# finsberg/fenicsx-beat

Hardware: AMD Instinct MI355X
Metric: node_updates_per_sec (higher is better)
Workload: dtype f64

## Files before the change

### fenicsx-beat_amd/csrc/beat_ode.hip

```cpp
#include "beat_ode_kernel.h"
#include "beat_ode_jit.h"

#include <functional>


template <class Model>
static int launch_ode_run(beat_ctx* ctx, double* states, int64_t n, int64_t ld, const double* host_params,
                          int num_params, const double* ppn, int64_t pld, double t0, double dt, int64_t nsteps,
                          int nbeats, int save_freq, const int* track_idx, int ntrack, double* trace) {
  BEAT_REQUIRE(num_params == Model::NP || (host_params == nullptr && ppn == nullptr && Model::NP == 2),
               "model expects %d parameters, got %d", Model::NP, num_params);
  BEAT_REQUIRE(ntrack >= 0 && ntrack <= 8, "at most 8 tracked states");
  BEAT_REQUIRE(ntrack == 0 || (trace != nullptr && save_freq >= 1), "tracking needs a trace buffer and save_freq >= 1");
  ParamPack<Model::NP> prm;
  for (int k = 0; k < Model::NP; ++k) prm.p[k] = host_params ? host_params[k] : 1.0;
  typename Model::Derived drv = Model::derive(prm.p);
  TrackSpec tr{};
  tr.n = ntrack;
  for (int a = 0; a < ntrack; ++a) {
    BEAT_REQUIRE(track_idx[a] >= 0 && track_idx[a] < Model::NS, "tracked state %d out of range", track_idx[a]);
    tr.idx[a] = track_idx[a];
  }
  const unsigned grid = (unsigned)((n + BEAT_BLOCK - 1) / BEAT_BLOCK);
  if (ppn != nullptr) {
    BEAT_REQUIRE(pld >= n, "params_ld %lld < n %lld", (long long)pld, (long long)n);
    BEAT_KERNEL((ode_run_kernel<Model, true>), dim3(grid), dim3(BEAT_BLOCK), 0, ctx->stream, states, n, ld, prm,
                       drv, ppn, pld, t0, dt, nsteps, nbeats, save_freq, tr, trace);
  } else {
    BEAT_KERNEL((ode_run_kernel<Model, false>), dim3(grid), dim3(BEAT_BLOCK), 0, ctx->stream, states, n, ld,
                       prm, drv, ppn, pld, t0, dt, nsteps, nbeats, save_freq, tr, trace);
  }
  BEAT_LAUNCH_CHECK();
  return BEAT_OK;
}

template <class M> struct ModelTag { using type = M; };
constexpr int BEAT_NOT_BUILTIN = 1001;

template <class F>
static int with_builtin_model(int model_id, F&& f) {
  switch (model_id) {
    case BEAT_MODEL_SIMPLE_ODE: return f(ModelTag<SimpleOde>{});
    case BEAT_MODEL_FHN_DEMO: return f(ModelTag<FhnDemo>{});
    case BEAT_MODEL_FHN_README: return f(ModelTag<FhnReadme>{});
    case BEAT_MODEL_TP06_GRL1: return f(ModelTag<Tp06Grl1>{});
    case BEAT_MODEL_TORORD_DYNCL_GRL1: return f(ModelTag<TorordDynClGrl1>{});
    case BEAT_MODEL_TORORD_LAND_GRL1: return f(ModelTag<TorordLandGrl1>{});
    default: return BEAT_NOT_BUILTIN;
  }
}

static int unknown_model(int model_id) {
  beat_set_error("unknown model id %d", model_id);
  return BEAT_EINVAL;
}

extern "C" int beat_ode_run(beat_ctx* ctx, int model_id, double* dev_states, int64_t n, int64_t ld,
                            const double* host_params, int num_params, const double* dev_params_per_node,
                            int64_t params_ld, double t0, double dt, int64_t nsteps, int nbeats, int save_freq,
                            const int* host_track_idx, int ntrack, double* dev_trace) {
  BEAT_REQUIRE(ctx != nullptr && dev_states != nullptr, "null argument");
  BEAT_REQUIRE(n >= 0 && ld >= n && nsteps >= 0 && nbeats >= 0, "bad shape");
  if (n == 0 || nsteps == 0 || nbeats == 0) return BEAT_OK;
  if (model_id >= BEAT_MODEL_CUSTOM_BASE)
    return beat_custom_run(ctx, model_id, dev_states, n, ld, host_params, num_params, dev_params_per_node, params_ld, t0, dt, nsteps, nbeats,
                           save_freq, host_track_idx, ntrack, dev_trace);
  const int rc = with_builtin_model(model_id, [&](auto tag) {
    return launch_ode_run<typename decltype(tag)::type>(ctx, dev_states, n, ld, host_params, num_params, dev_params_per_node, params_ld, t0, dt,
                                                        nsteps, nbeats, save_freq, host_track_idx, ntrack, dev_trace);
  });
  return rc == BEAT_NOT_BUILTIN ? unknown_model(model_id) : rc;
}

static unsigned ode_grid(int64_t n, int num_states) {
  unsigned grid = (unsigned)((n + BEAT_BLOCK - 1) / BEAT_BLOCK);
  static const int grid_cap_env = [] {
    const char* e = std::getenv("BEAT_ODE_GRID");
    return e ? std::atoi(e) : -1;
  }();
  static const int tile_min_states = [] {
    const char* e = std::getenv("BEAT_ODE_TILE_MIN_STATES");
    return e ? std::atoi(e) : 12;
  }();
  const int grid_cap = grid_cap_env >= 0 ? grid_cap_env : (num_states >= tile_min_states ? 0 : 24576);
  static const bool balance = [] {
    const char* e = std::getenv("BEAT_ODE_BALANCE");
    return !(e && e[0] == '0');
  }();
  if (grid_cap > 0 && grid > (unsigned)grid_cap) {
    const unsigned per_block = (grid + (unsigned)grid_cap - 1) / (unsigned)grid_cap;
    grid = (balance && per_block <= 8) ? (grid + per_block - 1) / per_block : (unsigned)grid_cap;
  }
  return grid;
}

template <class Model, bool PER_NODE, bool MARKED = false, bool SPARSE = false>
static auto launch_instance(bool have_pend, hipStream_t stream, unsigned grid, double* states, int64_t n, int64_t ld,
                            const ParamPack<Model::NP>& prm, const typename Model::Derived& drv, const double* ppn, int64_t pld, double t,
                            double dt, int v_index, double* v_copy, const PendingV& pend, const MarkedArgs& mk, const SparseRows& sp) {
  if (have_pend)
    BEAT_KERNEL((ode_step_kernel<Model, PER_NODE, true, MARKED, SPARSE>), dim3(grid), dim3(BEAT_BLOCK), 0, stream, states, n, ld, prm, drv,
                ppn, pld, t, dt, v_index, v_copy, pend, mk, sp);
  else
    BEAT_KERNEL((ode_step_kernel<Model, PER_NODE, false, MARKED, SPARSE>), dim3(grid), dim3(BEAT_BLOCK), 0, stream, states, n, ld, prm, drv,
                ppn, pld, t, dt, v_index, v_copy, pend, mk, sp);
}

template <class Model>
static int launch_ode(beat_ctx* ctx, double* states, int64_t n, int64_t ld, const double* host_params,
                      int num_params, const double* ppn, int64_t pld, double t, double dt,
                      int v_index, double* v_copy, const PendingV& pend, MarkedArgs mk = MarkedArgs{nullptr, nullptr, 0, nullptr, nullptr},
                      SparseRows sp = SparseRows{{0}, 0}) {
  BEAT_REQUIRE(num_params == Model::NP || (host_params == nullptr && ppn == nullptr && Model::NP == 2) || mk.markers != nullptr,
               "model expects %d parameters, got %d", Model::NP, num_params);
  BEAT_REQUIRE(host_params != nullptr || ppn != nullptr || mk.markers != nullptr || Model::NP == 2,
               "no parameters given: a host vector, per-node rows or parameter classes");
  if (int rc = beat_check_step_rows(Model::NS, Model::V_INDEX, v_index, v_copy, mk.markers != nullptr, pend)) return rc;
  const bool have_pend = beat_pending_has_work(pend);
  ParamPack<Model::NP> prm;
  for (int k = 0; k < Model::NP; ++k) prm.p[k] = host_params ? host_params[k] : 1.0;
  typename Model::Derived drv = Model::derive(prm.p);
  const unsigned grid = ode_grid(n, Model::NS);
  if (mk.markers != nullptr) {
    BEAT_REQUIRE(ppn == nullptr && mk.table != nullptr, "parameter classes come with a table, not with per-node rows");
    launch_instance<Model, false, true>(have_pend, ctx->stream, grid, states, n, ld, prm, drv, ppn, pld, t, dt, v_index, v_copy, pend, mk, sp);
  } else if (ppn != nullptr && sp.count > 0) {
    BEAT_REQUIRE(pld >= n, "params_ld %lld < n %lld", (long long)pld, (long long)n);
    BEAT_REQUIRE(host_params != nullptr, "sparse rows come with the uniform parameter vector");
    {
      const int rc = beat_ode_jit_launch<Model>(ctx, dim3(grid), have_pend, states, n, ld, prm, drv, ppn, pld, t, dt, v_index, v_copy, pend, mk, sp);
      if (rc != BEAT_JIT_UNAVAILABLE) return rc;
    }
    BEAT_REQUIRE(sp.count <= BEAT_MAX_SPARSE_ROWS_RT, "%d varying rows need run-time compilation, which is not available here "
                 "(beat_ode_jit_stats; at most %d rows otherwise): pass all rows (beat_ode_step)", sp.count, BEAT_MAX_SPARSE_ROWS_RT);
    launch_instance<Model, true, false, true>(have_pend, ctx->stream, grid, states, n, ld, prm, drv, ppn, pld, t, dt, v_index, v_copy, pend, mk,
                                              sp);
  } else if (ppn != nullptr) {
    BEAT_REQUIRE(pld >= n, "params_ld %lld < n %lld", (long long)pld, (long long)n);
    launch_instance<Model, true>(have_pend, ctx->stream, grid, states, n, ld, prm, drv, ppn, pld, t, dt, v_index, v_copy, pend, mk, sp);
  } else {
    launch_instance<Model, false>(have_pend, ctx->stream, grid, states, n, ld, prm, drv, ppn, pld, t, dt, v_index, v_copy, pend, mk, sp);
  }
  BEAT_LAUNCH_CHECK();
  return BEAT_OK;
}

extern "C" int beat_ode_model_info(int model_id, int* num_states, int* num_params) {
  int ns = 0, np = 0;
  const int rc = with_builtin_model(model_id, [&](auto tag) {
    using M = typename decltype(tag)::type;
    ns = M::NS;
    np = M::NP;
    return BEAT_OK;
  });
  if (rc == BEAT_NOT_BUILTIN && beat_custom_model_info(model_id, &ns, &np, nullptr) != BEAT_OK)
    return unknown_model(model_id);
  if (num_states) *num_states = ns;
  if (num_params) *num_params = np;
  return BEAT_OK;
}

static int ode_step_dispatch(beat_ctx* ctx, int model_id, double* dev_states, int64_t n, int64_t ld,
                             const double* host_params, int num_params, const double* dev_params_per_node,
                             int64_t params_ld, double t, double dt, int v_index, double* dev_v_copy,
                             const PendingV& pend, MarkedArgs mk = MarkedArgs{nullptr, nullptr, 0, nullptr, nullptr},
                             SparseRows sp = SparseRows{{0}, 0}) {
  BEAT_REQUIRE(ctx != nullptr, "null context");
  BEAT_REQUIRE(dev_states != nullptr, "null states");
  BEAT_REQUIRE(n >= 0 && ld >= n, "bad shape n=%lld ld=%lld", (long long)n, (long long)ld);
  BEAT_REQUIRE((n + BEAT_BLOCK - 1) / BEAT_BLOCK < (int64_t)0x7fffffff, "n too large");
  if (n == 0) return BEAT_OK;
  if (model_id >= BEAT_MODEL_CUSTOM_BASE) {
    BEAT_REQUIRE(sp.count == 0, "a model registered as source takes a uniform vector, all per-node rows or classes (no sparse rows)");
    int cns = 0, cnp = 0, cvi = 0;
    if (int rc = beat_custom_model_info(model_id, &cns, &cnp, &cvi)) return rc;
    return beat_custom_step(ctx, model_id, ode_grid(n, cns), dev_states, n, ld, host_params, num_params, dev_params_per_node, params_ld, t, dt,
                            v_index, dev_v_copy, pend, mk);
  }
  const int rc = with_builtin_model(model_id, [&](auto tag) {
    return launch_ode<typename decltype(tag)::type>(ctx, dev_states, n, ld, host_params, num_params, dev_params_per_node, params_ld, t, dt,
                                                    v_index, dev_v_copy, pend, mk, sp);
  });
  return rc == BEAT_NOT_BUILTIN ? unknown_model(model_id) : rc;
}

extern "C" int beat_ode_step(beat_ctx* ctx, int model_id, double* dev_states, int64_t n, int64_t ld,
                             const double* host_params, int num_params,
                             const double* dev_params_per_node, int64_t params_ld, double t, double dt,
                             int v_index, double* dev_v_copy) {
  return ode_step_dispatch(ctx, model_id, dev_states, n, ld, host_params, num_params, dev_params_per_node, params_ld,
                           t, dt, v_index, dev_v_copy, PendingV{nullptr, 0, nullptr, 0, {}});
}

static int flush_long_ring(beat_pde* pde, double* v_row, const double* dev_ring0, int64_t field_stride, int& pending) {
  if (pending <= BEAT_MAX_PENDING) return BEAT_OK;
  pending = 0;
  return beat_pde_x_flush_terms(pde, nullptr, v_row, dev_ring0, field_stride, pde->last_base, 0, pde->guess.take_pending());
}

static int step_behind_open_solve(beat_ctx* ctx, beat_pde* pde, const double* dev_ring0, int64_t field_stride, int64_t n, double* v_row,
                                  const std::function<int(const PendingV&)>& launch) {
  BEAT_REQUIRE(pde != nullptr && pde->open.on, "pending = -1 needs an operator with an open solve");
  BEAT_REQUIRE(dev_ring0 != nullptr && field_stride >= n, "bad pending update");
  BEAT_REQUIRE(pde->open.x == v_row, "the open solve does not work on this row");
  PendingV behind{dev_ring0, field_stride, pde->d_alphas, 0, pde->guess.cur, pde->d_st, pde->ring};
  if (int rc = launch(behind)) return rc;
  beat_ksp_info info{};
  int pend2[2] = {0, 0};
  bool needed_more = false;
  const int rc_solve = beat_solve_end(pde, 1, &info, pend2, &needed_more);
  if (rc_solve != BEAT_OK && rc_solve != BEAT_ENOTCONV) return rc_solve;
  pde->guess.applied_behind = false;
  if (!needed_more) {
    pde->guess.pending_applied_behind();
    return BEAT_OK;
  }
  return launch(PendingV{dev_ring0, field_stride, pend2[1] ? pde->d_alphas : nullptr, pend2[1], pde->guess.take_pending(), nullptr, 0});
}

static int step_with_pending(beat_ctx* ctx, beat_pde* pde, double* v_row, int64_t n, const double* dev_ring0, int64_t field_stride,
                             int pending, bool long_ring, bool node_map, const std::function<int(const PendingV&)>& launch) {
  static_assert(BEAT_MAX_PENDING == beat_pde_detail::PRING && BEAT_MAX_PENDING_CLASS == beat_pde_detail::PRING_MAX, "pending directions = ring size");
  if (pending == -1) {
    BEAT_REQUIRE(long_ring || (pde != nullptr && pde->ring <= BEAT_MAX_PENDING),
                 "this kernel's pending path takes %d directions: finish the solve first", BEAT_MAX_PENDING);
    return step_behind_open_solve(ctx, pde, dev_ring0, field_stride, node_map ? 0 : n, v_row, launch);
  }
  BEAT_REQUIRE(pending >= 0 && pending <= BEAT_MAX_PENDING_CLASS, "pending count %d out of range", pending);
  BEAT_REQUIRE(pending == 0 || (pde != nullptr && dev_ring0 != nullptr && (field_stride >= n || node_map)), "bad pending update");
  BEAT_REQUIRE(pde == nullptr || !pde->open.on, "the operator has an open solve: finish it (beat_pde_solve_end) or pass pending = -1");
  if (!long_ring)
    if (int rc = flush_long_ring(pde, v_row, dev_ring0, field_stride, pending)) return rc;
  PendingV pend{dev_ring0, field_stride, pending ? pde->d_alphas : nullptr, pending, {}};
  if (pde != nullptr) pend.gt = pde->guess.take_pending();
  return launch(pend);
}

extern "C" int beat_ode_step_pending(beat_ctx* ctx, int model_id, double* dev_states, int64_t n, int64_t ld,
                                     const double* host_params, int num_params,
                                     const double* dev_params_per_node, int64_t params_ld, double t, double dt,
                                     int v_index, double* dev_v_copy, beat_pde* pde, const double* dev_ring0,
                                     int64_t field_stride, int pending) {
  double* v_row = dev_states + (int64_t)v_index * ld;
  return step_with_pending(ctx, pde, v_row, n, dev_ring0, field_stride, pending, false, false,
                           [&](const PendingV& pv) {
    return ode_step_dispatch(ctx, model_id, dev_states, n, ld, host_params, num_params, dev_params_per_node, params_ld, t, dt, v_index,
                             dev_v_copy, pv);
  });
}


extern "C" int beat_ode_step_rows(beat_ctx* ctx, int model_id, double* dev_states, int64_t n, int64_t ld,
                                  const double* host_params, int num_params, const int* host_row_params, int num_rows,
                                  const double* dev_rows, int64_t rows_ld, double t, double dt, int v_index, double* dev_v_copy,
                                  beat_pde* pde, const double* dev_ring0, int64_t field_stride, int pending) {
  BEAT_REQUIRE(host_params != nullptr && host_row_params != nullptr && dev_rows != nullptr, "null argument");
  BEAT_REQUIRE(num_rows >= 1 && num_rows <= BEAT_MAX_SPARSE_ROWS, "1..%d varying rows, got %d", BEAT_MAX_SPARSE_ROWS, num_rows);
  BEAT_REQUIRE(num_rows <= BEAT_MAX_SPARSE_ROWS_RT || beat_jit_enabled(), "%d varying rows need run-time compilation, which is not available "
               "here (beat_ode_jit_stats; at most %d rows otherwise): pass all rows (beat_ode_step)", num_rows, BEAT_MAX_SPARSE_ROWS_RT);
  SparseRows sp{{0}, num_rows};
  for (int j = 0; j < num_rows; ++j) {
    BEAT_REQUIRE(host_row_params[j] >= 0 && host_row_params[j] < num_params, "row %d names parameter %d of %d", j, host_row_params[j], num_params);
    sp.idx[j] = host_row_params[j];
  }
  double* v_row = dev_states + (int64_t)v_index * ld;
  return step_with_pending(ctx, pde, v_row, n, dev_ring0, field_stride, pending, false, false,
                           [&](const PendingV& pv) {
    return ode_step_dispatch(ctx, model_id, dev_states, n, ld, host_params, num_params, dev_rows, rows_ld, t, dt, v_index, dev_v_copy, pv,
                             MarkedArgs{nullptr, nullptr, 0, nullptr, nullptr}, sp);
  });
}

template <class Model>
static int fill_table(const double* host_params, int num_params, int classes, std::vector<double>& out) {
  BEAT_REQUIRE(num_params == Model::NP, "model expects %d parameters, got %d", Model::NP, num_params);
  static_assert(sizeof(OdeTableEntry<Model>) % sizeof(double) == 0, "table entry is a whole number of doubles");
  const size_t stride = sizeof(OdeTableEntry<Model>) / sizeof(double);
  out.assign(stride * (size_t)classes, 0.0);
  for (int c = 0; c < classes; ++c) {
    OdeTableEntry<Model>* e = (OdeTableEntry<Model>*)(out.data() + stride * c);
    for (int k = 0; k < Model::NP; ++k) e->p[k] = host_params[(size_t)c * Model::NP + k];
    e->d = Model::derive(e->p);
  }
  return BEAT_OK;
}

extern "C" int beat_ode_class_table_doubles(int model_id, int* doubles_per_class) {
  BEAT_REQUIRE(doubles_per_class != nullptr, "null argument");
  const int rc = with_builtin_model(model_id, [&](auto tag) {
    *doubles_per_class = (int)(sizeof(OdeTableEntry<typename decltype(tag)::type>) / sizeof(double));
    return BEAT_OK;
  });
  if (rc != BEAT_NOT_BUILTIN) return rc;
  int np = 0;
// ... 151 lines not shown
```

### fenicsx-beat_amd/csrc/beat_ode_kernel.h

```cpp
#pragma once
#include "beat_pde_internal.h"

#include <algorithm>
#include <cmath>
#include <cstddef>
#include <cstdlib>
#include <type_traits>
#include <vector>
#include "ionic_models.h"
#include "torord_dyncl.h"


template <int NP>
struct ParamPack {
  double p[NP];
};

struct PendingV {
  const double* ring;
  int64_t fld;
  const double* alphas;
  int count;
  beat_pde_detail::GuessTerms gt;
  const double* dev_st;
  int ring_len;
};

struct PendingNow {
  int count;
  beat_pde_detail::GuessTerms gt;
};
__device__ __forceinline__ PendingNow beat_pending_now(const PendingV& p, int nupd) {
  PendingNow o{p.count, p.gt};
  if (nupd >= 0) {
    o.count = nupd % p.ring_len;
    o.gt.accumulate = nupd >= p.ring_len ? 1 : 0;
    const bool e_due = nupd == 0 && p.gt.use_e != 0;
    if (o.count == 0 && !e_due) o.gt.d = nullptr;
  }
  return o;
}

struct MarkedArgs {
  const unsigned char* markers;
  const double* table;
  int stride;
  const int* vmap;
  double* vfield;
};

template <class Model>
struct OdeStepKernArgHead {
  double* states;
  int64_t n, ld;
  ParamPack<Model::NP> prm;
  typename Model::Derived drv;
  const double* ppn;
  int64_t pld;
  double t, dt;
  int v_index;
  double* v_copy;
  PendingV pend;
  MarkedArgs mk;
};

constexpr int BEAT_MAX_SPARSE_ROWS = 16;
constexpr int BEAT_MAX_SPARSE_ROWS_RT = 4;
struct SparseRows {
  int idx[BEAT_MAX_SPARSE_ROWS];
  int count;
};

template <class Model>
struct OdeTableEntry {
  double p[Model::NP];
  typename Model::Derived d;
};

template <int... K>
struct IdxPack {
  static constexpr int count = (int)sizeof...(K);
};
template <class CT>
struct MixedParams;
template <int... K>
struct MixedParams<IdxPack<K...>> {
  const double* u;
  double v[sizeof...(K) > 0 ? sizeof...(K) : 1];
  __device__ __forceinline__ double operator[](int k) const {
    double r = u[k];
    int j = 0;
    ((r = (k == K ? v[j] : r), ++j), ...);
    return r;
  }
};
template <class D, unsigned long long DM0, unsigned long long DM1>
__device__ __forceinline__ D mix_derived(const D& du, const D& dl) {
  D d;
  constexpr int ND = (int)(sizeof(D) / sizeof(double));
  static_assert(sizeof(D) % sizeof(double) == 0 && ND <= 128, "Derived: up to 128 doubles");
  const double* a = (const double*)&du;
  const double* b = (const double*)&dl;
  double* o = (double*)&d;
#pragma unroll
  for (int j = 0; j < ND; ++j) o[j] = (((j < 64 ? DM0 : DM1) >> (j & 63)) & 1ull) ? b[j] : a[j];
  return d;
}

template <class Model, class = void>
struct beat_fm_type { using type = FastMath; };
template <class Model>
struct beat_fm_type<Model, std::void_t<typename Model::FM>> { using type = typename Model::FM; };
template <class Model, class = void>
struct beat_fm_pin_wanted : std::false_type {};
template <class Model>
struct beat_fm_pin_wanted<Model, std::void_t<decltype(Model::FM_PIN)>> : std::integral_constant<bool, Model::FM_PIN> {};
__device__ __forceinline__ double beat_any_value() {
  double x;
#ifdef __AMDGCN__
  asm volatile("" : "=v"(x));
#else
  x = 0.0;
#endif
  return x;
}
template <class Model, bool PER_NODE, bool PEND, bool MARKED = false, bool SPARSE = false, class CT = IdxPack<>,
          unsigned long long DM0 = 0, unsigned long long DM1 = 0>
__global__ __launch_bounds__(BEAT_BLOCK, (PER_NODE && CT::count == 0) ? Model::WAVES_PER_NODE : Model::WAVES) void ode_step_kernel(
    double* __restrict__ states, int64_t n, int64_t ld, ParamPack<Model::NP> prm,
    typename Model::Derived drv, const double* __restrict__ ppn, int64_t pld, double t, double dt,
    int v_index, double* __restrict__ v_copy, PendingV pend, MarkedArgs mk_arg, SparseRows sp) {
  __shared__ double etab[BEAT_EXP_TAB];
  __shared__ LogEntry ltab[128];
  static_assert(BEAT_EXP_TAB == BEAT_BLOCK, "one table entry per thread");
  etab[threadIdx.x] = beat_exp_tab_entry<beat_fm_type<Model>::type::INT_SCALE>(kExp2Tab[threadIdx.x], (int)threadIdx.x);
  if (threadIdx.x < 128) ltab[threadIdx.x] = kLogTab[threadIdx.x];
  __shared__ int cls_jn[MARKED ? BEAT_BLOCK : 1];
  __shared__ int s_pend[2];
  if (PEND && threadIdx.x == 0) {
    s_pend[0] = pend.dev_st != nullptr ? (pend.dev_st[beat_pde_detail::STOP] != 0.0 ? 1 : 0) : 1;
    s_pend[1] = pend.dev_st != nullptr ? (int)pend.dev_st[beat_pde_detail::NUPD] : -1;
  }
  __syncthreads();
  typename beat_fm_type<Model>::type fm{etab, ltab};
  if constexpr (beat_fm_pin_wanted<Model>::value) beat_fm_pin(fm);
  if (PEND && s_pend[0] == 0) return;
  const int wave_in_block = __builtin_amdgcn_readfirstlane((int)(threadIdx.x >> 6));
  for (int64_t tile = blockIdx.x;; tile += gridDim.x) {
  typedef const __attribute__((address_space(4))) char* KArgPtr;
  KArgPtr ka = (KArgPtr)__builtin_amdgcn_kernarg_segment_ptr();
  asm volatile("" : "+s"(ka));
  const PendingV& pendl = *(const PendingV*)(ka + offsetof(OdeStepKernArgHead<Model>, pend));
  const OdeStepKernArgHead<Model>& hd = *(const OdeStepKernArgHead<Model>*)ka;
  double* __restrict__ const states = hd.states;
  const int64_t n = hd.n, ld = hd.ld;
  const double* __restrict__ const ppn = hd.ppn;
  const int64_t pld = hd.pld;
  const double t = hd.t, dt = hd.dt;
  const int v_index = hd.v_index;
  double* __restrict__ const v_copy = hd.v_copy;
  (void)ppn; (void)pld; (void)v_index; (void)v_copy;
  if (tile * BEAT_BLOCK >= n) break;
  int lane_now = (int)__builtin_amdgcn_mbcnt_hi(~0u, __builtin_amdgcn_mbcnt_lo(~0u, 0u));
  asm volatile("" : "+v"(lane_now));
  const int tid = (wave_in_block << 6) + lane_now;
  const int64_t tile0 = tile * BEAT_BLOCK;
  unsigned lane_off = (unsigned)tid * 8u;
  const int64_t i = tile0 + tid;
  if (i >= n) break;
  int64_t ldl = ld;
  asm volatile("" : "+s"(ldl));
  if (MARKED) {
    const MarkedArgs& mk = *(const MarkedArgs*)(ka + offsetof(OdeStepKernArgHead<Model>, mk));
    const int m_lane = mk.markers[i];
    const int64_t jn = mk.vmap != nullptr ? (int64_t)mk.vmap[i] : i;
    double* const vptr = mk.vmap != nullptr ? mk.vfield + jn : states + (int64_t)Model::V_INDEX * ld + i;
    if (mk.vmap != nullptr) cls_jn[tid] = (int)jn;
    struct NodeIOWithV {
      double* __restrict__ base;
      int64_t ld;
      mutable unsigned i;
      double* vbase;
      const int* jn_slot;
      double v;
      __device__ __forceinline__ double load(int k) const { return k == Model::V_INDEX ? v : beat_row_load(beat_at(beat_row(base, k, ld), i)); }
      __device__ __forceinline__ void store(int k, double x) const {
        beat_row_store(beat_at(beat_row(base, k, ld), i), x);
        if (k == Model::V_INDEX && vbase != nullptr) {
          if (jn_slot != nullptr)
            vbase[*(const int*)((const char*)jn_slot + (i >> 1))] = x;
          else
            *beat_at(vbase, i) = x;
        }
      }
    };
    double v_now = m_lane != 254 ? *vptr : 0.0;
    if (PEND && m_lane != 254) {
      const PendingNow now = beat_pending_now(pendl, __builtin_amdgcn_readfirstlane(*(volatile int*)&s_pend[1]));
      double pp[BEAT_MAX_PENDING_CLASS], pa[BEAT_MAX_PENDING_CLASS];
#pragma unroll
      for (int j = 0; j < BEAT_MAX_PENDING_CLASS; ++j) {
        pp[j] = j < now.count ? __builtin_nontemporal_load(pendl.ring + (int64_t)j * pendl.fld + jn) : 0.0;
        pa[j] = j < now.count ? pendl.alphas[j] : 0.0;
      }
      if (now.gt.d != nullptr) {
        const beat_pde_detail::GuessTerms& gt = now.gt;
        const double ge = beat_pde_detail::beat_guess_needs_e(gt) ? __builtin_nontemporal_load(gt.e + jn) : 0.0;
        const double gd = beat_pde_detail::beat_guess_needs_d(gt) ? __builtin_nontemporal_load(gt.d + jn) : 0.0;
        const double gp0 = beat_pde_detail::beat_guess_needs_dp(gt, 0) ? __builtin_nontemporal_load(gt.dp[0] + jn) : 0.0;
        const double gp1 = beat_pde_detail::beat_guess_needs_dp(gt, 1) ? __builtin_nontemporal_load(gt.dp[1] + jn) : 0.0;
        double inc = gt.accumulate ? 0.0 : ge;
#pragma unroll
        for (int j = 0; j < BEAT_MAX_PENDING_CLASS; ++j)
          if (j < now.count) inc = fma(pa[j], pp[j], inc);
        beat_pde_detail::beat_guess_record(gt, gt.d + jn, gt.e + jn, inc, gd, gp0, gp1, ge);
        v_now += inc;
      } else {
#pragma unroll
        for (int j = 0; j < BEAT_MAX_PENDING_CLASS; ++j)
          if (j < now.count) v_now = fma(pa[j], pp[j], v_now);
      }
    }
    if (PEND && m_lane == 255) {
      *vptr = v_now;
      if (mk.vmap != nullptr) states[(int64_t)Model::V_INDEX * ld + i] = v_now;
    }
    unsigned long long todo = __ballot(m_lane < 254);
    while (todo) {
      const int m = __builtin_amdgcn_readlane(m_lane, __ffsll((long long)todo) - 1);
      typedef const __attribute__((address_space(4))) char* TabPtr;
      TabPtr tb = (TabPtr)(uintptr_t)(mk.table + (int64_t)m * mk.stride);
      asm volatile("" : "+s"(tb));
      const double* p_c = (const double*)(tb + offsetof(OdeTableEntry<Model>, p));
      const typename Model::Derived& d_c = *(const typename Model::Derived*)(tb + offsetof(OdeTableEntry<Model>, d));
      asm volatile("" : "+s"(ldl));
      NodeIOWithV iol{states + tile0, ldl, lane_off, mk.vmap != nullptr ? mk.vfield : (v_copy != nullptr ? v_copy + tile0 : nullptr),
                      mk.vmap != nullptr ? cls_jn : nullptr, v_now};
      asm volatile("" : "+v"(iol.i), "+v"(iol.v));
      if (m_lane == m) Model::step(iol, p_c, d_c, fm, t, dt);
      todo &= ~__ballot(m_lane == m);
    }
    continue;
  }
  const double* p_uni = (const double*)(ka + offsetof(OdeStepKernArgHead<Model>, prm));
  const typename Model::Derived& d_uni =
      *(const typename Model::Derived*)(ka + offsetof(OdeStepKernArgHead<Model>, drv));
  if (PEND) {
    PendingNow now = beat_pending_now(pendl, __builtin_amdgcn_readfirstlane(*(volatile int*)&s_pend[1]));
    NodeIOPending<Model::V_INDEX> io{states + tile0, ldl, lane_off, v_copy != nullptr ? v_copy + tile0 : nullptr, now.count, {}, {}, 0.0, 0.0, 0.0, 0.0, {}};
#pragma unroll
    for (int j = 0; j < BEAT_MAX_PENDING; ++j) {
      io.pp[j] = j < now.count ? __builtin_nontemporal_load(beat_at(pendl.ring + ((int64_t)j * pendl.fld + tile0), lane_off)) : beat_any_value();
      io.pa[j] = j < now.count ? pendl.alphas[j] : 0.0;
    }
    io.ge = io.gd = io.gp0 = io.gp1 = 0.0;
    if (now.gt.d != nullptr) {
      now.gt.d += tile0;
      now.gt.e += tile0;
      if (now.gt.dp[0] != nullptr) now.gt.dp[0] += tile0;
      if (now.gt.dp[1] != nullptr) now.gt.dp[1] += tile0;
      io.gt = now.gt;
      io.ge = beat_pde_detail::beat_guess_needs_e(now.gt) ? __builtin_nontemporal_load(beat_at(now.gt.e, lane_off)) : beat_any_value();
      io.gd = beat_pde_detail::beat_guess_needs_d(now.gt) ? __builtin_nontemporal_load(beat_at(now.gt.d, lane_off)) : beat_any_value();
      io.gp0 = beat_pde_detail::beat_guess_needs_dp(now.gt, 0) ? __builtin_nontemporal_load(beat_at(now.gt.dp[0], lane_off)) : beat_any_value();
      io.gp1 = beat_pde_detail::beat_guess_needs_dp(now.gt, 1) ? __builtin_nontemporal_load(beat_at(now.gt.dp[1], lane_off)) : beat_any_value();
    }
    if constexpr (PER_NODE && SPARSE && CT::count > 0) {
      MixedParams<CT> mp;
      mp.u = p_uni;
#pragma unroll
      for (int j = 0; j < CT::count; ++j) mp.v[j] = *beat_at(beat_row(ppn + tile0, j, pld), lane_off);
      if constexpr (DM0 == 0 && DM1 == 0) {
        Model::step(io, mp, d_uni, fm, t, dt);
      } else {
        const typename Model::Derived dlane = Model::derive(mp);
        const typename Model::Derived dm = mix_derived<typename Model::Derived, DM0, DM1>(d_uni, dlane);
        Model::step(io, mp, dm, fm, t, dt);
      }
    } else if (PER_NODE) {
      double pl[Model::NP];
      if (SPARSE) {
        const double* pv = p_uni;
        asm volatile("" : "+v"(pv));
#pragma unroll
        for (int k = 0; k < Model::NP; ++k) pl[k] = pv[k];
#pragma unroll
        for (int j = 0; j < BEAT_MAX_SPARSE_ROWS_RT; ++j) {
          if (j < sp.count) {
            const double vj = *beat_at(beat_row(ppn + tile0, j, pld), lane_off);
            int ij = sp.idx[j];
            asm volatile("" : "+s"(ij));
#pragma unroll
            for (int k = 0; k < Model::NP; ++k) pl[k] = k == ij ? vj : pl[k];
          }
        }
      } else {
#pragma unroll
        for (int k = 0; k < Model::NP; ++k) pl[k] = *beat_at(beat_row(ppn + tile0, k, pld), lane_off);
      }
      const typename Model::Derived dl = Model::derive(pl);
      Model::step(io, pl, dl, fm, t, dt);
    } else {
      Model::step(io, p_uni, d_uni, fm, t, dt);
    }
  } else {
    const NodeIO io{states + tile0, ldl, lane_off, nullptr, -1};
    if constexpr (PER_NODE && SPARSE && CT::count > 0) {
      MixedParams<CT> mp;
      mp.u = p_uni;
#pragma unroll
      for (int j = 0; j < CT::count; ++j) mp.v[j] = *beat_at(beat_row(ppn + tile0, j, pld), lane_off);
      if constexpr (DM0 == 0 && DM1 == 0) {
        Model::step(io, mp, d_uni, fm, t, dt);
      } else {
        const typename Model::Derived dlane = Model::derive(mp);
        const typename Model::Derived dm = mix_derived<typename Model::Derived, DM0, DM1>(d_uni, dlane);
        Model::step(io, mp, dm, fm, t, dt);
      }
    } else if (PER_NODE) {
      double pl[Model::NP];
      if (SPARSE) {
        const double* pv = p_uni;
        asm volatile("" : "+v"(pv));
#pragma unroll
        for (int k = 0; k < Model::NP; ++k) pl[k] = pv[k];
#pragma unroll
        for (int j = 0; j < BEAT_MAX_SPARSE_ROWS_RT; ++j) {
          if (j < sp.count) {
            const double vj = *beat_at(beat_row(ppn + tile0, j, pld), lane_off);
            int ij = sp.idx[j];
            asm volatile("" : "+s"(ij));
#pragma unroll
            for (int k = 0; k < Model::NP; ++k) pl[k] = k == ij ? vj : pl[k];
          }
        }
      } else {
#pragma unroll
        for (int k = 0; k < Model::NP; ++k) pl[k] = *beat_at(beat_row(ppn + tile0, k, pld), lane_off);
      }
      const typename Model::Derived dl = Model::derive(pl);
      Model::step(io, pl, dl, fm, t, dt);
    } else {
      Model::step(io, p_uni, d_uni, fm, t, dt);
    }
    if (v_copy != nullptr) v_copy[i] = states[(int64_t)v_index * ldl + i];
  }
  }
}

struct TrackSpec {
  int idx[8];
  int n;
};

template <class Model, bool PER_NODE>
__global__ __launch_bounds__(BEAT_BLOCK, 1) void ode_run_kernel(
    double* __restrict__ states, int64_t n, int64_t ld, ParamPack<Model::NP> prm, typename Model::Derived drv,
    const double* __restrict__ ppn, int64_t pld, double t0, double dt, int64_t nsteps, int nbeats, int save_freq,
    TrackSpec track, double* __restrict__ trace) {
  __shared__ double etab[BEAT_EXP_TAB];
  __shared__ LogEntry ltab[128];
  static_assert(BEAT_EXP_TAB == BEAT_BLOCK, "one table entry per thread");
  etab[threadIdx.x] = beat_exp_tab_entry<beat_fm_type<Model>::type::INT_SCALE>(kExp2Tab[threadIdx.x], (int)threadIdx.x);
  if (threadIdx.x < 128) ltab[threadIdx.x] = kLogTab[threadIdx.x];
  __syncthreads();
  typename beat_fm_type<Model>::type fm{etab, ltab};
  if constexpr (beat_fm_pin_wanted<Model>::value) beat_fm_pin(fm);
  const int64_t i = (int64_t)blockIdx.x * BEAT_BLOCK + threadIdx.x;
  if (i >= n) return;
  double y[Model::NS];
#pragma unroll
  for (int k = 0; k < Model::NS; ++k) y[k] = states[(int64_t)k * ld + i];
  double pl[PER_NODE ? Model::NP : 1];
  typename Model::Derived dl = drv;
  if (PER_NODE) {
#pragma unroll
    for (int k = 0; k < Model::NP; ++k) pl[k] = ppn[(int64_t)k * pld + i];
    dl = Model::derive((const double*)pl);
  }
  const RegIO rio{y};
  const NodeIO gio{states + (int64_t)blockIdx.x * BEAT_BLOCK, ld, threadIdx.x * 8u, nullptr, -1};
  int64_t row = 0;
  for (int beat = 0; beat < nbeats; ++beat) {
    for (int64_t j = 0; j < nsteps; ++j) {
      if (track.n > 0 && j % save_freq == 0) {
        for (int a = 0; a < track.n; ++a) {
          double v = 0.0;
#pragma unroll
          for (int k = 0; k < Model::NS; ++k)
            if (k == track.idx[a]) v = y[k];
          trace[(row * track.n + a) * n + i] = v;
        }
        ++row;
      }
      const double t = t0 + (double)j * dt;
      if (Model::REGISTER_LOOP) {
        if (PER_NODE)
          Model::step(rio, (const double*)pl, dl, fm, t, dt);
        else
          Model::step(rio, prm.p, dl, fm, t, dt);
// ... 78 lines not shown
```

### fenicsx-beat_amd/csrc/ionic_models.h

```cpp
#pragma once

#include <cmath>
#include <type_traits>
#include <utility>

#include "beat_common.h"


constexpr int BEAT_EXP_TAB = 256;
__device__ const double kExp2Tab[BEAT_EXP_TAB] = {
    1.0, 1.0027112750502025, 1.0054299011128027, 1.0081558981184175,
    1.0108892860517005, 1.0136300849514894, 1.016378314910953, 1.019133996077738,
    1.0218971486541166, 1.0246677928971357, 1.0274459491187637, 1.030231637686041,
    1.0330248790212284, 1.0358256936019572, 1.0386341019613787, 1.041450124688316,
    1.0442737824274138, 1.0471050958792898, 1.0499440858006872, 1.0527907730046264,
    1.0556451783605572, 1.0585073227945128, 1.061377227289262, 1.0642549128844645,
    1.0671404006768237, 1.0700337118202419, 1.0729348675259756, 1.075843889062791,
    1.0787607977571199, 1.0816856149932152, 1.0846183622133092, 1.0875590609177697,
    1.0905077326652577, 1.0934643990728858, 1.0964290818163769, 1.099401802630222,
    1.102382583307841, 1.1053714457017412, 1.1083684117236787, 1.1113735033448175,
    1.1143867425958924, 1.1174081515673693, 1.1204377524096067, 1.12347556733302,
    1.1265216186082418, 1.129575928566288, 1.1326385195987192, 1.1357094141578055,
    1.1387886347566916, 1.1418762039695616, 1.1449721444318042, 1.148076478840179,
    1.1511892299529827, 1.154310420590216, 1.1574400736337511, 1.1605782120274988,
// ... 233 lines not shown
  return std::isfinite(x) ? (std::frexp(x, &e), e) : 0;
#endif
}
__device__ __forceinline__ bool beat_pos_finite(double x) {
#ifdef __AMDGCN__
  return __builtin_amdgcn_class(x, 0x180);
#else
  return x > 0.0 && x < HUGE_VAL;
#endif
}
__device__ __forceinline__ double beat_log_special(double x) {
  const double y = x + 0.0;
  return y - __builtin_amdgcn_rsq(y);
}

__device__ __forceinline__ double beat_sconst(double c) {
#ifdef __AMDGCN__
  asm volatile("" : "+s"(c));
#endif
  return c;
}

template <bool INT_SCALE_>
struct FastMathT {
  static constexpr bool INT_SCALE = INT_SCALE_;
  const double* __restrict__ tab;
  const LogEntry* __restrict__ ltab;
  double magic = 6755399441055744.0;
  __device__ __forceinline__ double log(double x) const {
    const double xm = beat_frexp_mant(x);
    const int hi = __double2hiint(xm);
    const int e = beat_frexp_exp(x) - 1;
    const LogEntry t = ltab[(hi >> 13) & 127];
    const double m = __hiloint2double((hi & 0x000fffff) | 0x3ff00000, __double2loint(xm));
    const double r = fma(m, t.inv, -1.0);
    double p = fma(r, -1.0 / 6.0, 1.0 / 5.0);
    p = fma(r, p, -0.25);
    p = fma(r, p, 1.0 / 3.0);
    p = fma(r, p, -0.5);
    p = fma(r * r, p, r);
    const double ed = (double)e;
    const double es = __hiloint2double(beat_pos_finite(x) ? __double2hiint(ed) : __double2hiint(beat_log_special(x)), __double2loint(ed));
    return fma(es, 0.693147180559663, t.logc + fma(es, 2.8235290563031577e-13, p));
  }
  __device__ __forceinline__ double exp(double x) const {
    const double kb = fma(x, 369.3299304675746, magic);
    const double k = kb - magic;
    double r = fma(k, -0.002707606173999011, x);
    r = fma(k, -6.327543041662719e-14, r);
    const int ki = __double2loint(kb);
    const double t = tab[ki & (BEAT_EXP_TAB - 1)];
    const double r2 = r * r;
    double p = fma(r, beat_sconst(1.0 / 6.0), 0.5);
    p = fma(r2, beat_sconst(1.0 / 24.0), p);
    p = fma(r2, p, r);
#ifdef __AMDGCN__
    if constexpr (INT_SCALE) {
      const double ts = __hiloint2double(__double2hiint(t) + (int)((unsigned)ki << 12), __double2loint(t));
      return fma(ts, p, ts);
    }
#endif
    return ldexp(fma(t, p, t), ki >> 8);
  }
};

using FastMath = FastMathT<false>;
template <bool I>
__device__ __forceinline__ void beat_fm_pin(FastMathT<I>& fm) {
#ifdef __AMDGCN__
  asm volatile("" : "+v"(fm.magic));
#endif
}

__device__ __forceinline__ double beat_guard(double v) { return fabs(v) < 1.0e-4 ? copysign(1.0e-4, v) : v; }

__device__ __forceinline__ double beat_row_load(const double* p) {
#ifdef __clang__
  return __builtin_nontemporal_load(p);
#else
  return *p;
#endif
}
__device__ __forceinline__ void beat_row_store(double* p, double v) {
#ifdef __clang__
  __builtin_nontemporal_store(v, p);
#else
  *p = v;
#endif
}

template <class T>
__device__ __forceinline__ T* beat_row(T* base, int k, int64_t ld) {
#ifdef __AMDGCN__
  asm volatile("" : "+s"(ld));
#endif
  return base + (int64_t)k * ld;
}
template <class T>
__device__ __forceinline__ T* beat_at(T* uniform_base, unsigned& byte_off) {
  typedef typename std::conditional<std::is_const<T>::value, const char, char>::type Byte;
#ifdef __AMDGCN__
  asm volatile("" : "+v"(byte_off));
#endif
  return (T*)((Byte*)uniform_base + byte_off);
}
struct NodeIO {
  double* __restrict__ base;
  int64_t ld;
  mutable unsigned i;
  double* __restrict__ v_copy;
  int v_index;
  __device__ __forceinline__ double load(int k) const { return beat_row_load(beat_at(beat_row(base, k, ld), i)); }
  __device__ __forceinline__ void store(int k, double v) const {
    beat_row_store(beat_at(beat_row(base, k, ld), i), v);
    if (v_copy != nullptr && k == v_index) *beat_at(v_copy, i) = v;
  }
};

constexpr int BEAT_MAX_PENDING = 6;
constexpr int BEAT_MAX_PENDING_CLASS = 12;
template <int VIDX>
struct NodeIOPending {
  double* __restrict__ base;
  int64_t ld;
  mutable unsigned i;
  double* __restrict__ v_copy;
  int npend;
  double pa[BEAT_MAX_PENDING], pp[BEAT_MAX_PENDING];
  double ge, gd, gp0, gp1;
  beat_pde_detail::GuessTerms gt;
  __device__ __forceinline__ double load(int k) const {
    double x = beat_row_load(beat_at(beat_row(base, k, ld), i));
    if (k == VIDX) {
      if (gt.d != nullptr) {
        double inc = (!gt.accumulate && gt.use_e) ? ge : 0.0;
#pragma unroll
        for (int j = 0; j < BEAT_MAX_PENDING; ++j)
          if (j < npend) inc = fma(pa[j], pp[j], inc);
        beat_pde_detail::beat_guess_record(gt, beat_at(gt.d, i), beat_at(gt.e, i), inc, gd, gp0, gp1, ge);
        return x + inc;
      }
#pragma unroll
      for (int j = 0; j < BEAT_MAX_PENDING; ++j)
        if (j < npend) x = fma(pa[j], pp[j], x);
    }
    return x;
  }
  __device__ __forceinline__ void store(int k, double v) const {
    beat_row_store(beat_at(beat_row(base, k, ld), i), v);
    if (k == VIDX && v_copy != nullptr) *beat_at(v_copy, i) = v;
  }
};

struct RegIO {
  double* y;
  __device__ __forceinline__ double load(int k) const { return y[k]; }
  __device__ __forceinline__ void store(int k, double v) const { y[k] = v; }
};

struct SimpleOde {
  static constexpr int NS = 2, NP = 2, V_INDEX = 0;
  static constexpr bool REGISTER_LOOP = true;
  static constexpr int WAVES = BEAT_ODE_WAVES;
  static constexpr int WAVES_PER_NODE = BEAT_ODE_WAVES_PER_NODE;
  struct Derived {};
  __host__ __device__ static Derived derive(const double*) { return {}; }
  template <class IO>
  __device__ static __forceinline__ void step(const IO& io, const double* p, const Derived&, const FastMath&,
                                              double, double dt) {
    const double v = io.load(0), s = io.load(1);
    io.store(0, v - p[0] * s * dt);
    io.store(1, s + p[1] * v * dt);
  }
};

struct FhnDemo {
  static constexpr int NS = 2, NP = 10, V_INDEX = 1;
  static constexpr bool REGISTER_LOOP = true;
  static constexpr int WAVES = BEAT_ODE_WAVES;
  static constexpr int WAVES_PER_NODE = BEAT_ODE_WAVES_PER_NODE;
  struct Derived {};
  __host__ __device__ static Derived derive(const double*) { return {}; }
  template <class IO>
  __device__ static __forceinline__ void step(const IO& io, const double* p, const Derived&, const FastMath&,
                                              double t, double dt) {
    const double s = io.load(0), V = io.load(1);
    const double V_peak = p[0], V_rest = p[1], a = p[2], b = p[3], c_1 = p[4], c_2 = p[5],
                 c_3 = p[6], stim_amplitude = p[7], stim_duration = p[8], stim_start = p[9];
    const double V_amp = V_peak - V_rest;
    const double i_Stim = (t >= stim_start && t <= stim_start + stim_duration) ? stim_amplitude : 0.0;
    const double ds_dt = b * (-c_3 * s + (V - V_rest));
    const double V_th = V_amp * a + V_rest;
    const double I = -s * (c_2 / V_amp) * (V - V_rest) +
                     (((c_1 / (V_amp * V_amp)) * (V - V_rest)) * (V - V_th)) * (-V + V_peak);
    const double dV_dt = I + i_Stim;
    io.store(0, s + dt * ds_dt);
    io.store(1, V + dt * dV_dt);
  }
};

struct FhnReadme {
  static constexpr int NS = 2, NP = 11, V_INDEX = 1;
  static constexpr bool REGISTER_LOOP = true;
  static constexpr int WAVES = BEAT_ODE_WAVES;
  static constexpr int WAVES_PER_NODE = BEAT_ODE_WAVES_PER_NODE;
  struct Derived {};
  __host__ __device__ static Derived derive(const double*) { return {}; }
  template <class IO>
  __device__ static __forceinline__ void step(const IO& io, const double* p, const Derived&, const FastMath&,
                                              double t, double dt) {
    const double s = io.load(0), v = io.load(1);
    const double c_1 = p[0], c_2 = p[1], c_3 = p[2], a = p[3], b = p[4], v_amp = p[5],
                 v_rest = p[6], v_peak = p[7], stim_amplitude = p[8], stim_duration = p[9],
                 stim_start = p[10];
    const double i_app = (t > stim_start && t < stim_start + stim_duration) ? stim_amplitude : 0.0;
    const double ds_dt = b * (-c_3 * s + (v - v_rest));
    const double v_th = v_amp * a + v_rest;
    const double I = -s * (c_2 / v_amp) * (v - v_rest) +
                     (((c_1 / (v_amp * v_amp)) * (v - v_rest)) * (v - v_th)) * (-v + v_peak);
    const double dV_dt = I + i_app;
    io.store(0, ds_dt * dt + s);
    io.store(1, v + dV_dt * dt);
  }
};

#ifdef __clang__
#pragma clang fp contract(fast)
#endif
struct Tp06Grl1 {
  static constexpr int NS = 19, NP = 53, V_INDEX = 17;
  static constexpr bool ACCESSOR_PARAMS = true;
  static constexpr bool REGISTER_LOOP = true;
#ifndef BEAT_TP06_WAVES
#define BEAT_TP06_WAVES 4
#endif
  static constexpr int WAVES = BEAT_TP06_WAVES;
  static constexpr int WAVES_PER_NODE = BEAT_ODE_WAVES_PER_NODE;
  using FM = FastMath;
  static constexpr bool FM_PIN = true;
  enum S { Xr1, Xr2, Xs, m, h, j, d, f, f2, fCass, s, r, R_prime, Ca_i, Ca_SR, Ca_ss, Na_i, V, K_i };
  enum P {
    P_kna, g_K1, g_Kr, g_Ks, g_Na, g_bna, g_CaL, g_bca, g_to, P_NaK, K_mk, K_mNa, K_NaCa, K_sat,
    alpha, gamma, Km_Ca, Km_Nai, g_pCa, K_pCa, g_pK, Ca_o, k1_prime, k2_prime, k3, k4, EC, max_sr,
    min_sr, V_rel, V_xfer, K_up, V_leak, Vmax_up, Buf_c, K_buf_c, Buf_sr, K_buf_sr, Buf_ss,
    K_buf_ss, V_sr, V_ss, Na_o, R, T, F, Cm, V_c, stim_start, stim_period, stim_duration,
    stim_amplitude, K_o
  };

  struct Derived {
    double RTF, FRT, halfRTF, sqrtKo, gK1s, gKrs, KoPk, cCaL, NaK_B, Nao3, A2c, kNaCaQ, gm1,
        cVF, c1, c2, c3, c4, c5, Kup2, BKc, BKsr, BKss, dsr;
  };
  template <class P>
  __host__ __device__ static Derived derive(const P& p) {
    Derived q;
    q.RTF = p[R] * p[T] / p[F];
    q.FRT = p[F] / (p[R] * p[T]);
    q.halfRTF = 0.5 * p[R] * p[T] / p[F];
    q.sqrtKo = sqrt(p[K_o] / 5.4);
    q.gK1s = p[g_K1] * q.sqrtKo;
    q.gKrs = p[g_Kr] * q.sqrtKo;
    q.KoPk = p[K_o] + p[P_kna] * p[Na_o];
    q.cCaL = p[g_CaL] * 4.0 * (p[F] * p[F]) / (p[R] * p[T]);
    q.NaK_B = p[P_NaK] * p[K_o] / (p[K_o] + p[K_mk]);
    q.Nao3 = p[Na_o] * p[Na_o] * p[Na_o];
    q.A2c = q.Nao3 * p[alpha];
    q.kNaCaQ = p[K_NaCa] / ((p[Km_Nai] * p[Km_Nai] * p[Km_Nai] + q.Nao3) * (p[Km_Ca] + p[Ca_o]));
    q.gm1 = p[gamma] - 1.0;
    q.cVF = p[Cm] / (p[V_c] * p[F]);
    q.c1 = p[Cm] / (2.0 * p[V_c] * p[F]);
    q.c2 = p[V_sr] / p[V_c];
    q.c3 = p[Cm] / (2.0 * p[V_ss] * p[F]);
    q.c4 = p[V_sr] / p[V_ss];
    q.c5 = p[V_c] / p[V_ss];
    q.Kup2 = p[K_up] * p[K_up];
    q.BKc = p[Buf_c] * p[K_buf_c];
    q.BKsr = p[Buf_sr] * p[K_buf_sr];
    q.BKss = p[Buf_ss] * p[K_buf_ss];
    q.dsr = p[max_sr] - p[min_sr];
    return q;
  }

  __device__ static __forceinline__ double rcp(double x) { return beat_rcp(x); }
  __device__ static __forceinline__ void rcp2(double a, double b, double& ia, double& ib) {
    const double r = rcp(a * b);
    ia = r * b;
    ib = r * a;
  }
  __device__ static __forceinline__ void rcp3(double a, double b, double c, double& ia, double& ib, double& ic) {
    const double ab = a * b;
    const double r = rcp(ab * c);
    ic = r * ab;
    const double t = r * c;
    ia = t * b;
    ib = t * a;
  }
  __device__ static __forceinline__ void rcp4(double a, double b, double c, double d, double& ia, double& ib,
                                              double& ic, double& id) {
    const double ab = a * b, cd = c * d;
    const double r = rcp(ab * cd);
    const double rab = r * cd, rcd = r * ab;
    ia = rab * b;
    ib = rab * a;
    ic = rcd * d;
    id = rcd * c;
  }
  __device__ static __forceinline__ double grl1(const FM& fm, double y, double fy, double J, double dt) {
    return y + ((fabs(J) > 1e-8) ? fy * (beat_exp_overflow(J * dt, fm.exp(beat_clamp_exp_arg<FM::INT_SCALE>(J * dt))) - 1.0) * rcp(J) : fy * dt);
  }
  __device__ static __forceinline__ double phi_small(double z) {
    double ph = fma(z, beat_sconst(1.0 / 362880.0), beat_sconst(1.0 / 40320.0));
    ph = fma(z, ph, beat_sconst(1.0 / 5040.0));
    ph = fma(z, ph, beat_sconst(1.0 / 720.0));
    ph = fma(z, ph, beat_sconst(1.0 / 120.0));
    ph = fma(z, ph, beat_sconst(1.0 / 24.0));
    ph = fma(z, ph, beat_sconst(1.0 / 6.0));
    ph = fma(z, ph, 0.5);
    return fma(z, ph, 1.0);
  }
  __device__ static __forceinline__ double advance(const FM& fm, double y, double fy, double J, double dt) {
    const double z = J * dt;
    if (fabs(z) <= 0.0625) return fma(fy * dt, phi_small(z), y);
    return grl1(fm, y, fy, J, dt);
  }
  __device__ static __forceinline__ double phi7(double z) {
    double ph = fma(z, beat_sconst(1.0 / 40320.0), beat_sconst(1.0 / 5040.0));
    ph = fma(z, ph, beat_sconst(1.0 / 720.0));
    ph = fma(z, ph, beat_sconst(1.0 / 120.0));
    ph = fma(z, ph, beat_sconst(1.0 / 24.0));
    ph = fma(z, ph, beat_sconst(1.0 / 6.0));
    ph = fma(z, ph, 0.5);
    return fma(z, ph, 1.0);
  }
  __device__ static __forceinline__ double gate(const FM& fm, double y, double inf, double rtau, double dt) {
    return y + (inf - y) * (1.0 - fm.exp(fmax(-dt * rtau, BEAT_EXP_LO)));
  }

#define BEAT_FENCE() __builtin_amdgcn_sched_barrier(0)

  template <class IO, class P>
  __device__ static __forceinline__ void step(const IO& io, const P& p, const Derived& q, const FM& fm,
                                              double t, double dt) {
    const double v = io.load(V);
    constexpr double EXP_M3 = 0.049787068367863944;
    constexpr double EXP_2P5 = 12.182493960703473;
    constexpr double EXP_M4P5 = 0.011108996538242306;
    constexpr double EXP_1P3 = 3.6692966676192444;
    constexpr double EXP_3 = 20.085536923187668;
    constexpr double EXP_M3P2 = 0.04076220397836621;
    constexpr double EXP_M12 = 6.14421235332821e-06;
    constexpr double EXP_7 = 1096.6331584284585;
    constexpr double EXP_1 = 2.718281828459045;
    constexpr double EXP_4 = 54.598150033144236;
    constexpr double EXP_M4 = 0.01831563888873418;
    constexpr double EXP_M26_7 = 0.0243728440732796;
    constexpr double EXP_20_7 = 17.41170806332765;
    constexpr double EXP_5 = 148.4131591025766;
    constexpr double EXP_5_6 = 2.300975890892825;
    constexpr double EXP_20_6 = 28.03162489452614;
    constexpr double EXP_M1 = 0.36787944117144233;
    constexpr double EXP_P02 = 1.0202013400267558;

    const double oXr1 = io.load(Xr1), oXr2 = io.load(Xr2), oXs = io.load(Xs), om = io.load(m), oh = io.load(h),
                 oj = io.load(j), od = io.load(d), of = io.load(f), of2 = io.load(f2), ofCass = io.load(fCass),
                 os = io.load(s), orr = io.load(r);
    const double gNa = p[g_Na] * (om * om * om) * oh * oj;
    const double gKr = q.gKrs * oXr1 * oXr2;
    const double gKs = p[g_Ks] * (oXs * oXs);
    const double gto = p[g_to] * orr * os;
    const double gates_CaL = q.cCaL * od * of * of2 * ofCass;
    const double vCai = io.load(Ca_i), vCaSR = io.load(Ca_SR), vCass = io.load(Ca_ss), vNai = io.load(Na_i),
                 vKi = io.load(K_i), vR = io.load(R_prime);

    const double E20 = fm.exp(0.05 * v), E7 = fm.exp(v * (1.0 / 7.0));
    double I20, I7;
    rcp2(E20, E7, I20, I7);
    const double E10 = E20 * E20, I10 = I20 * I20;
    const double E5 = E10 * E10, I5 = I10 * I10;
    const double I6 = fm.exp(v * (-1.0 / 6.0));
    BEAT_FENCE();

    {
      double inf1, inf2;
      rcp2(1.0 + EXP_M26_7 * I7, 1.0 + fm.exp((v + 88.0) * (1.0 / 24.0)), inf1, inf2);
      const double rtau1 = (1.0 + EXP_M4P5 * I10) * (1.0 + fm.exp((v + 30.0) * (1.0 / 11.5))) * (1.0 / 2700.0);
// ... 237 lines not shown
```

Before: 11.55 billion.

## Preload all state rows into registers at kernel entry for TP06 uniform-parameter path

```diff
diff --git a/fenicsx-beat_amd/csrc/beat_ode.hip b/fenicsx-beat_amd/csrc/beat_ode.hip
--- a/fenicsx-beat_amd/csrc/beat_ode.hip
+++ b/fenicsx-beat_amd/csrc/beat_ode.hip
@@ -139,7 +139,9 @@
     BEAT_REQUIRE(pld >= n, "params_ld %lld < n %lld", (long long)pld, (long long)n);
     launch_instance<Model, true>(have_pend, ctx->stream, grid, states, n, ld, prm, drv, ppn, pld, t, dt, v_index, v_copy, pend, mk, sp);
   } else {
-    launch_instance<Model, false>(have_pend, ctx->stream, grid, states, n, ld, prm, drv, ppn, pld, t, dt, v_index, v_copy, pend, mk, sp);
+    const unsigned tiles = (unsigned)((n + BEAT_BLOCK - 1) / BEAT_BLOCK);
+    launch_instance<Model, false>(have_pend, ctx->stream, (beat_rows_preloaded<Model>::value && !have_pend) ? tiles : grid, states, n, ld, prm, drv, ppn, pld, t,
+                                  dt, v_index, v_copy, pend, mk, sp);
   }
   BEAT_LAUNCH_CHECK();
   return BEAT_OK;
diff --git a/fenicsx-beat_amd/csrc/beat_ode_kernel.h b/fenicsx-beat_amd/csrc/beat_ode_kernel.h
--- a/fenicsx-beat_amd/csrc/beat_ode_kernel.h
+++ b/fenicsx-beat_amd/csrc/beat_ode_kernel.h
@@ -115,6 +115,22 @@
 struct beat_fm_pin_wanted : std::false_type {};
 template <class Model>
 struct beat_fm_pin_wanted<Model, std::void_t<decltype(Model::FM_PIN)>> : std::integral_constant<bool, Model::FM_PIN> {};
+template <class Model, class = void>
+struct beat_rows_preloaded : std::false_type {};
+template <class Model>
+struct beat_rows_preloaded<Model, std::void_t<decltype(Model::PRELOAD_ROWS)>> : std::integral_constant<bool, Model::PRELOAD_ROWS> {};
+template <class Model>
+__device__ __forceinline__ void beat_load_rows(double (&y)[Model::NS], const double* tile_base, int64_t ld, unsigned& lane_off) {
+  y[Model::V_INDEX] = beat_row_load(beat_at(beat_row(tile_base, Model::V_INDEX, ld), lane_off));
+#pragma unroll
+  for (int k = 0; k < Model::NS; ++k)
+    if (k != Model::V_INDEX) y[k] = beat_row_load(beat_at(beat_row(tile_base, k, ld), lane_off));
+}
+__device__ __forceinline__ void beat_under_branch(double& x) {
+#ifdef __AMDGCN__
+  asm volatile("" : "+v"(x));
+#endif
+}
 __device__ __forceinline__ double beat_any_value() {
   double x;
 #ifdef __AMDGCN__
@@ -130,6 +146,14 @@
     double* __restrict__ states, int64_t n, int64_t ld, ParamPack<Model::NP> prm,
     typename Model::Derived drv, const double* __restrict__ ppn, int64_t pld, double t, double dt,
     int v_index, double* __restrict__ v_copy, PendingV pend, MarkedArgs mk_arg, SparseRows sp) {
+  constexpr bool ROWS_BY_KERNEL = beat_rows_preloaded<Model>::value && !PER_NODE && !MARKED;
+  constexpr bool ROWS_AHEAD = ROWS_BY_KERNEL && !PEND;
+  double rows_ahead[ROWS_AHEAD ? Model::NS : 1];
+  if constexpr (ROWS_AHEAD) {
+    const int64_t tile_first = (int64_t)blockIdx.x * BEAT_BLOCK;
+    unsigned off_first = threadIdx.x * 8u;
+    if (tile_first + threadIdx.x < n) beat_load_rows<Model>(rows_ahead, states + tile_first, ld, off_first);
+  }
   __shared__ double etab[BEAT_EXP_TAB];
   __shared__ LogEntry ltab[128];
   static_assert(BEAT_EXP_TAB == BEAT_BLOCK, "one table entry per thread");
@@ -245,7 +269,72 @@
   const double* p_uni = (const double*)(ka + offsetof(OdeStepKernArgHead<Model>, prm));
   const typename Model::Derived& d_uni =
       *(const typename Model::Derived*)(ka + offsetof(OdeStepKernArgHead<Model>, drv));
-  if (PEND) {
+  if constexpr (ROWS_BY_KERNEL) {
+    NodeIOLoaded<Model::NS, Model::V_INDEX> io{states + tile0, ldl, lane_off, (PEND && v_copy != nullptr) ? v_copy + tile0 : nullptr, {}};
+    if constexpr (ROWS_AHEAD) {
+#pragma unroll
+      for (int k = 0; k < Model::NS; ++k) io.y[k] = rows_ahead[k];
+    } else {
+      io.y[Model::V_INDEX] = beat_row_load(beat_at(beat_row(io.base, Model::V_INDEX, ldl), io.i));
+    }
+    if (PEND) {
+      typedef volatile __attribute__((address_space(3))) int* LdsInt;
+      PendingNow now = beat_pending_now(pendl, __builtin_amdgcn_readfirstlane(*(LdsInt)&s_pend[1]));
+      double pp[BEAT_MAX_PENDING], pa[BEAT_MAX_PENDING];
+#pragma unroll
+      for (int j = 0; j < BEAT_MAX_PENDING; ++j) {
+        pp[j] = j < now.count ? __builtin_nontemporal_load(beat_at(pendl.ring + ((int64_t)j * pendl.fld + tile0), io.i)) : beat_any_value();
+        pa[j] = j < now.count ? pendl.alphas[j] : 0.0;
+      }
+      const beat_pde_detail::GuessTerms& gt = now.gt;
+      const bool guess = gt.d != nullptr;
+      double* const gd_p = gt.d + tile0;
+      double* const ge_p = gt.e + tile0;
+      const double ge = guess && beat_pde_detail::beat_guess_needs_e(gt) ? __builtin_nontemporal_load(beat_at((const double*)ge_p, io.i)) : 0.0;
+      const double gd = guess && beat_pde_detail::beat_guess_needs_d(gt) ? __builtin_nontemporal_load(beat_at((const double*)gd_p, io.i)) : 0.0;
+      const double gp0 = guess && beat_pde_detail::beat_guess_needs_dp(gt, 0) ? __builtin_nontemporal_load(beat_at(gt.dp[0] + tile0, io.i)) : 0.0;
+      const double gp1 = guess && beat_pde_detail::beat_guess_needs_dp(gt, 1) ? __builtin_nontemporal_load(beat_at(gt.dp[1] + tile0, io.i)) : 0.0;
+#pragma unroll
+      for (int k = 0; k < Model::NS; ++k)
+        if (k != Model::V_INDEX) io.y[k] = beat_row_load(beat_at(beat_row(io.base, k, ldl), io.i));
+#ifdef __AMDGCN__
+      static_assert(Model::NS - 1 <= 63, "vmcnt has six bits");
+      __builtin_amdgcn_s_waitcnt(0x0F70 | ((Model::NS - 1) & 15) | (((Model::NS - 1) >> 4) << 14));
+#endif
+      double& v = io.y[Model::V_INDEX];
+      if (guess) {
+        double inc = (!gt.accumulate && gt.use_e) ? ge : 0.0;
+#pragma unroll
+        for (int j = 0; j < BEAT_MAX_PENDING; ++j) {
+          if (j >= now.count) break;
+          inc = fma(pa[j], pp[j], inc);
+          beat_under_branch(inc);
+        }
+        if (gt.accumulate) {
+          *beat_at(gd_p, io.i) = gd + inc;
+          *beat_at(ge_p, io.i) = fma(gt.a, inc, ge);
+        } else {
+          double en = gt.a * inc;
+          if (gt.cp[0] != 0.0) en = fma(gt.cp[0], gp0, en), beat_under_branch(en);
+          if (gt.cp[1] != 0.0) en = fma(gt.cp[1], gp1, en), beat_under_branch(en);
+          if (gt.cd != 0.0) en = fma(gt.cd, gd, en), beat_under_branch(en);
+          *beat_at(gd_p, io.i) = inc;
+          *beat_at(ge_p, io.i) = en;
+        }
+        v = v + inc;
+      } else {
+#pragma unroll
+        for (int j = 0; j < BEAT_MAX_PENDING; ++j) {
+          if (j >= now.count) break;
+          v = fma(pa[j], pp[j], v);
+          beat_under_branch(v);
+        }
+      }
+    }
+    Model::step(io, p_uni, d_uni, fm, t, dt);
+    if (!PEND && v_copy != nullptr) *beat_at(v_copy + tile0, io.i) = *beat_at(beat_row(io.base, v_index, ldl), io.i);
+    if constexpr (ROWS_AHEAD) break;
+  } else if (PEND) {
     PendingNow now = beat_pending_now(pendl, __builtin_amdgcn_readfirstlane(*(volatile int*)&s_pend[1]));
     NodeIOPending<Model::V_INDEX> io{states + tile0, ldl, lane_off, v_copy != nullptr ? v_copy + tile0 : nullptr, now.count, {}, {}, 0.0, 0.0, 0.0, 0.0, {}};
 #pragma unroll
diff --git a/fenicsx-beat_amd/csrc/ionic_models.h b/fenicsx-beat_amd/csrc/ionic_models.h
--- a/fenicsx-beat_amd/csrc/ionic_models.h
+++ b/fenicsx-beat_amd/csrc/ionic_models.h
@@ -409,6 +409,20 @@
   }
 };
 
+template <int NS, int VIDX>
+struct NodeIOLoaded {
+  double* __restrict__ base;
+  int64_t ld;
+  mutable unsigned i;
+  double* __restrict__ v_copy;
+  double y[NS];
+  __device__ __forceinline__ double load(int k) const { return y[k]; }
+  __device__ __forceinline__ void store(int k, double v) const {
+    beat_row_store(beat_at(beat_row(base, k, ld), i), v);
+    if (k == VIDX && v_copy != nullptr) *beat_at(v_copy, i) = v;
+  }
+};
+
 struct RegIO {
   double* y;
   __device__ __forceinline__ double load(int k) const { return y[k]; }
@@ -488,6 +502,7 @@
   static constexpr int NS = 19, NP = 53, V_INDEX = 17;
   static constexpr bool ACCESSOR_PARAMS = true;
   static constexpr bool REGISTER_LOOP = true;
+  static constexpr bool PRELOAD_ROWS = true;
 #ifndef BEAT_TP06_WAVES
 #define BEAT_TP06_WAVES 4
 #endif
```

New measurement: 11.67 billion, median of 6. 1.0% higher.
